# Adttil/crypto12381

Measured on AMD Instinct MI355X. Metric: G1 scalar-muls/s per MI355X (batch 2^20 per GPU), bit-exact vs CPU, higher is better.
Workload: dtype int64 accumulate over 14x28-bit signed limbs

## Files before the change

### crypto12381_amd/csrc/consts.hpp

```cpp
#pragma once
#include <cstdint>

namespace c12381 {

constexpr int NL = 14;
constexpr int LB = 28;
constexpr uint32_t LMASK = 0xfffffffu;
constexpr uint32_t FP_N0 = 0xffcfffdu;

C12381_CONST int32_t FP_P[14] = {0xfffaaab, 0xfefffff, 0x3ffffb9, 0xfffeb15, 0x6241eab, 0xa0f6b0f, 0xf6730d2, 0xf38512b, 0x4774b84, 0x4bacd76, 0xba7b643, 0xe69a4b1, 0x1ea397f, 0x001a011};
C12381_CONST int32_t FP_R1[14] = {0x347fcb8, 0xd800000, 0x002b119, 0x0cde6d2, 0xc7212e0, 0x83a2090, 0x037669f, 0xda0f73e, 0x9b09b42, 0x1297bb0, 0x515d98f, 0x012ca7c, 0x659fcfa, 0x000577a};
C12381_CONST int32_t FP_R2[14] = {0x10370ed, 0x6d1c345, 0xe243d62, 0xec45c53, 0x3b1d65a, 0x093317d, 0xb4f36a0, 0x5d74088, 0xc10ea72, 0x865d118, 0x7320a75, 0xfd5cd50, 0xcc8a759, 0x000c8d4};
C12381_CONST int32_t SG_P30[13] = {0x3fffaaab, 0x27fbffff, 0x153ffffb, 0x2affffac, 0x30f6241e, 0x034a83da, 0x112bf673, 0x12e13ce1, 0x2cd76477, 0x1ed90d2e, 0x29a4b1ba, 0x3a8e5ff9, 0x001a0111};
constexpr uint32_t SG_PINV30 = 0x30003u;
C12381_CONST int32_t FP_B3[14] = {0x760834a, 0x2200002, 0x8204dc2, 0x9a6fbad, 0x910a528, 0xe9ab0aa, 0x3ca6dd4, 0x51af490, 0xb58b018, 0x47c315a, 0x5b6c62e, 0x40e3470, 0x86368b8, 0x000d99a};
C12381_CONST int32_t FP_FOUR[14] = {0xd1ff2e0, 0x6000000, 0x00ac467, 0x3379b48, 0x1c84b80, 0x0e88243, 0x0dd9a7e, 0x683dcf8, 0x6c26d0b, 0x4a5eec2, 0x457663c, 0x04b29f1, 0x967f3e8, 0x0015de9};
C12381_CONST int32_t FP_HALF[14] = {0x1a3fe5c, 0xec00000, 0x001588c, 0x066f369, 0x6390970, 0xc1d1048, 0x01bb34f, 0x6d07b9f, 0x4d84da1, 0x894bdd8, 0x28aecc7, 0x009653e, 0x32cfe7d, 0x0002bbd};
C12381_CONST int32_t FP_INV3[14] = {0x66d1b5a, 0x4755555, 0x2ab902f, 0x0449454, 0x2e8c568, 0x972fce5, 0xa5742c1, 0x405dddc, 0x63510c4, 0x8dfb234, 0x977175c, 0x44cb14a, 0x8ba2553, 0x0013289};
C12381_CONST int32_t FP_BETA_A[14] = {0xa75929a, 0x681b798, 0x22a3e9d, 0xabc02bf, 0x4e5bb45, 0x55e6e7e, 0x4814117, 0x6d04f1b, 0xae3387d, 0x54acb0c, 0x0a4c74b, 0x56138b5, 0xb64e066, 0x00076f2};
C12381_CONST int32_t FP_BETA_B[14] = {0x2421b59, 0xbee4867, 0x1d31002, 0x4760184, 0x4cc5086, 0xc76dc00, 0xaae891b, 0xac70ad2, 0xfe377c4, 0xe4686b8, 0x5ed1568, 0x8f5a180, 0x02b5c1f, 0x000d1a4};
C12381_CONST int32_t FROB_F_A[14] = {0x9f1ba38, 0xed52b31, 0x3131f18, 0x932815a, 0x35bde3f, 0x7c4a4df, 0xc6f7465, 0x266b7cc, 0x2acd4ff, 0xcae398d, 0x243b688, 0xa613121, 0x72d376f, 0x0001c3e};
C12381_CONST int32_t FROB_F_B[14] = {0x60df073, 0x11ad4ce, 0x0ece0a1, 0x6cd69bb, 0x2c8406c, 0x24ac630, 0x2f7bc6d, 0xcd1995f, 0x1ca7685, 0x80c93e9, 0x963ffba, 0x4087390, 0xabd0210, 0x00183d2};
C12381_CONST int32_t FROB_F2_A[14] = {0x0000000, 0x0000000, 0x0000000, 0x0000000, 0x0000000, 0x0000000, 0x0000000, 0x0000000, 0x0000000, 0x0000000, 0x0000000, 0x0000000, 0x0000000, 0x0000000};
C12381_CONST int32_t FROB_F2_B[14] = {0x2421b59, 0xbee4867, 0x1d31002, 0x4760184, 0x4cc5086, 0xc76dc00, 0xaae891b, 0xac70ad2, 0xfe377c4, 0xe4686b8, 0x5ed1568, 0x8f5a180, 0x02b5c1f, 0x000d1a4};
C12381_CONST int32_t FROB_F3_A[14] = {0x33e2f27, 0x32a25aa, 0x27ca1d2, 0xc1e049e, 0xc3f707a, 0x055ca94, 0x2010b7b, 0x3b93794, 0xd5a86aa, 0xa544de3, 0x556a044, 0x9c66da5, 0x38ec515, 0x000cea3};
C12381_CONST int32_t FROB_F3_B[14] = {0x33e2f27, 0x32a25aa, 0x27ca1d2, 0xc1e049e, 0xc3f707a, 0x055ca94, 0x2010b7b, 0x3b93794, 0xd5a86aa, 0xa544de3, 0x556a044, 0x9c66da5, 0x38ec515, 0x000cea3};
C12381_CONST int32_t PSI1_X_A[14] = {0x0000000, 0x0000000, 0x0000000, 0x0000000, 0x0000000, 0x0000000, 0x0000000, 0x0000000, 0x0000000, 0x0000000, 0x0000000, 0x0000000, 0x0000000, 0x0000000};
C12381_CONST int32_t PSI1_X_B[14] = {0x58a1811, 0x96e4867, 0x1d5c11c, 0x543e856, 0x13e6366, 0x4b0fc91, 0xae5efbb, 0x8680210, 0x9941307, 0xf700269, 0xb02eef7, 0x9086bfc, 0x6855919, 0x001291e};
C12381_CONST int32_t PSI1_Y_A[14] = {0xcc17b84, 0xcc5da55, 0x1835de7, 0x3e1e677, 0x9e4ae31, 0x9b9a07a, 0xd662557, 0xb7f1997, 0x71cc4da, 0xa667f92, 0x65115fe, 0x4a3370c, 0xe5b746a, 0x000d16d};
C12381_CONST int32_t PSI1_Y_B[14] = {0x33e2f27, 0x32a25aa, 0x27ca1d2, 0xc1e049e, 0xc3f707a, 0x055ca94, 0x2010b7b, 0x3b93794, 0xd5a86aa, 0xa544de3, 0x556a044, 0x9c66da5, 0x38ec515, 0x000cea3};
C12381_CONST int32_t PSI3_X_A[14] = {0x0000000, 0x0000000, 0x0000000, 0x0000000, 0x0000000, 0x0000000, 0x0000000, 0x0000000, 0x0000000, 0x0000000, 0x0000000, 0x0000000, 0x0000000, 0x0000000};
C12381_CONST int32_t PSI3_X_B[14] = {0xcb7adf3, 0x26fffff, 0x3fd4ea0, 0xf320443, 0x9b20bcb, 0x1d54a7e, 0xf2fca33, 0x19759ed, 0xac6b042, 0x39151c5, 0x691dcb4, 0xe56da35, 0xb903c85, 0x0014896};
C12381_CONST int32_t PSI3_Y_A[14] = {0x33e2f27, 0x32a25aa, 0x27ca1d2, 0xc1e049e, 0xc3f707a, 0x055ca94, 0x2010b7b, 0x3b93794, 0xd5a86aa, 0xa544de3, 0x556a044, 0x9c66da5, 0x38ec515, 0x000cea3};
// ... 97 lines not shown
```

### crypto12381_amd/csrc/fp.hpp

```cpp
#pragma once
#include <cstdint>
#include <type_traits>
#include <utility>

#if defined(__HIPCC__)
#include <hip/hip_runtime.h>
#define C12381_HD __host__ __device__ __forceinline__
#define C12381_HDN __host__ __device__ __noinline__ inline
#define C12381_CONST __device__ constexpr
#else
#define C12381_HD inline
#define C12381_HDN inline
#define C12381_CONST constexpr
#endif

#if defined(__HIP_DEVICE_COMPILE__)
#define C12381_LIMB(x) c12381::limb_opaque(x)
namespace c12381 { __device__ __forceinline__ int32_t limb_opaque(int32_t v) { asm("" : "+v"(v)); return v; } }
#else
#define C12381_LIMB(x) (x)
#endif

#include "consts.hpp"

// ... 17 lines not shown

struct fp {
    int32_t l[NL];
#ifdef C12381_CHECK_BOUNDS
    double lb = 0, vb = 0;
#endif
};

#ifdef C12381_CHECK_BOUNDS
inline void bounds_fail(const char* what, double a, double b) {
    std::fprintf(stderr, "C12381 bound violation: %s (%.4g, %.4g)\n", what, a, b);
    void* frames[48];
    int nf = backtrace(frames, 48);
    backtrace_symbols_fd(frames, nf, 2);
    std::abort();
}
constexpr double P_OVER_R = 0.000396;
constexpr double TOP_PER_P = 106514.0;
inline void check_actual(const fp& a, const char* where) {
    for (int i = 0; i < NL; ++i)
        if (std::fabs((double)a.l[i]) > a.lb) bounds_fail(where, (double)a.l[i], a.lb);
}
inline void check_actual_vb(const fp& a, const char* where);
inline void set_inj_bounds(fp& r, double sum_lblb, double sum_vbvb, double inj_abs, double inj_lb, const char* where);
inline void set_bounds(fp& r, double lb, double vb, const char* where) {
    r.lb = lb; r.vb = vb;
    if (lb > 2147483648.0) bounds_fail("limb bound exceeds int32", lb, vb);
    check_actual(r, where);
}
#endif

C12381_HD void fp_add(fp& r, const fp& a, const fp& b) {
#pragma unroll
    for (int i = 0; i < NL; ++i) r.l[i] = a.l[i] + b.l[i];
    C12381_BOUNDS(set_bounds(r, a.lb + b.lb, a.vb + b.vb, "fp_add");)
}
C12381_HD void fp_sub(fp& r, const fp& a, const fp& b) {
#pragma unroll
    for (int i = 0; i < NL; ++i) r.l[i] = a.l[i] - b.l[i];
    C12381_BOUNDS(set_bounds(r, a.lb + b.lb, a.vb + b.vb, "fp_sub");)
}
C12381_HD void fp_neg(fp& r, const fp& a) {
#pragma unroll
    for (int i = 0; i < NL; ++i) r.l[i] = -a.l[i];
    C12381_BOUNDS(set_bounds(r, a.lb, a.vb, "fp_neg");)
}
C12381_HD void fp_dbl(fp& r, const fp& a) { fp_add(r, a, a); }
// ... 39 lines not shown
    t += (int64_t)a.l[NL - 1] * k;
    r.l[NL - 1] = (int32_t)t;
    C12381_BOUNDS({ double top = a.vb * k * TOP_PER_P + 2.0;
                    set_bounds(r, top > 268435456.0 ? top : 268435456.0, a.vb * k, "fp_mul_small"); })
}

C12381_HD void fp_weak_reduce(fp& r, const fp& a) {
    fp n;
    fp_norm1(n, a);
    const int32_t q = (int32_t)(((int64_t)n.l[NL - 1] * 40324 + ((int64_t)1 << 31)) >> 32);
    int64_t t = 0;
#pragma unroll
    for (int i = 0; i < NL - 1; ++i) {
        t += (int64_t)n.l[i] - (int64_t)q * FP_P[i];
        r.l[i] = C12381_LIMB((int32_t)((uint32_t)t & LMASK));
        t >>= LB;
    }
    t += (int64_t)n.l[NL - 1] - (int64_t)q * FP_P[NL - 1];
    r.l[NL - 1] = (int32_t)t;
    C12381_BOUNDS({ if (a.vb > 2400.0) bounds_fail("fp_weak_reduce input value bound", a.vb, 0);
                    set_bounds(r, 268435456.0, 1.6, "fp_weak_reduce"); })
}

#ifdef C12381_CHECK_BOUNDS
inline void check_mul_operands(const fp& a, const fp& b, const char* where) {
    check_actual(a, where); check_actual(b, where);
    double col = 14.0 * a.lb * b.lb + 14.0 * 72057594037927936.0 + 1099511627776.0;
    if (col >= 9223372036854775808.0) bounds_fail(where, a.lb, b.lb);
    if (a.vb * b.vb > 1.0e6) bounds_fail("fp_mul value bound", a.vb, b.vb);
}
#endif

C12381_HD void fp_mul(fp& r, const fp& a, const fp& b) {
    C12381_BOUNDS(check_mul_operands(a, b, "fp_mul");)
    C12381_COUNT(27, 1);
    int32_t m[NL];
    int32_t out[NL];
    int64_t acc = 0;
#pragma unroll
    for (int k = 0; k < NL; ++k) {
#pragma unroll
        for (int i = 0; i <= k; ++i) { acc += (int64_t)a.l[i] * b.l[k - i]; }
#pragma unroll
        for (int i = 0; i < k; ++i) { acc += (int64_t)m[i] * FP_P[k - i]; }
        m[k] = (int32_t)(((uint32_t)acc * FP_N0) & LMASK);
        acc += (int64_t)m[k] * FP_P[0];
        acc >>= LB;
    }
#pragma unroll
    for (int k = NL; k < 2 * NL - 1; ++k) {
#pragma unroll
        for (int i = k - NL + 1; i < NL; ++i) { acc += (int64_t)a.l[i] * b.l[k - i]; }
#pragma unroll
        for (int i = k - NL + 1; i < NL; ++i) { acc += (int64_t)m[i] * FP_P[k - i]; }
        out[k - NL] = C12381_LIMB((int32_t)((uint32_t)acc & LMASK));
        acc >>= LB;
    }
    out[NL - 1] = (int32_t)acc;
#pragma unroll
    for (int i = 0; i < NL; ++i) r.l[i] = out[i];
    C12381_BOUNDS({ double vb = a.vb * b.vb * P_OVER_R + 1.0;
                    double top = vb * TOP_PER_P + 2.0;
                    set_bounds(r, top > 268435456.0 ? top : 268435456.0, vb, "fp_mul"); })
}

C12381_HD void fp_sqr(fp& r, const fp& a) {
    C12381_BOUNDS(check_mul_operands(a, a, "fp_sqr");)
    C12381_COUNT(27, 1);
    int32_t m[NL];
    int32_t out[NL];
    int32_t a2[NL];
#pragma unroll
    for (int i = 0; i < NL; ++i) a2[i] = 2 * a.l[i];
    int64_t acc = 0;
#pragma unroll
    for (int k = 0; k < NL; ++k) {
#pragma unroll
        for (int i = 0; 2 * i < k; ++i) { acc += (int64_t)a2[i] * a.l[k - i]; }
        if ((k & 1) == 0) { acc += (int64_t)a.l[k / 2] * a.l[k / 2]; }
#pragma unroll
        for (int i = 0; i < k; ++i) { acc += (int64_t)m[i] * FP_P[k - i]; }
        m[k] = (int32_t)(((uint32_t)acc * FP_N0) & LMASK);
        acc += (int64_t)m[k] * FP_P[0];
        acc >>= LB;
    }
#pragma unroll
    for (int k = NL; k < 2 * NL - 1; ++k) {
#pragma unroll
        for (int i = k - NL + 1; 2 * i < k; ++i) { acc += (int64_t)a2[i] * a.l[k - i]; }
        if ((k & 1) == 0) { acc += (int64_t)a.l[k / 2] * a.l[k / 2]; }
#pragma unroll
        for (int i = k - NL + 1; i < NL; ++i) { acc += (int64_t)m[i] * FP_P[k - i]; }
        out[k - NL] = C12381_LIMB((int32_t)((uint32_t)acc & LMASK));
        acc >>= LB;
    }
    out[NL - 1] = (int32_t)acc;
#pragma unroll
    for (int i = 0; i < NL; ++i) r.l[i] = out[i];
    C12381_BOUNDS({ double vb = a.vb * a.vb * P_OVER_R + 1.0;
                    double top = vb * TOP_PER_P + 2.0;
                    set_bounds(r, top > 268435456.0 ? top : 268435456.0, vb, "fp_sqr"); })
}

C12381_HD void fp_col_acc(int64_t& acc, const fp& a, const fp& b, int k) {
    C12381_COUNT(1, 0);
#pragma unroll
    for (int i = 0; i < NL; ++i) {
        const int j = k - i;
        if (j >= 0 && j < NL) { acc += (int64_t)a.l[i] * b.l[j]; }
    }
}
C12381_HD void fp_col_sqr_acc(int64_t& acc, const fp& a, const fp& a2, const fp& ad, int k) {
    C12381_COUNT(1, 0);
#pragma unroll
    for (int i = 0; i < NL; ++i) {
        const int j = k - i;
        if (j > i && j < NL) { acc += (int64_t)a2.l[i] * a.l[j]; }
    }
    if ((k & 1) == 0 && k / 2 < NL) { acc += (int64_t)ad.l[k / 2] * a.l[k / 2]; }
}
C12381_HD void fp_raw_neg(fp& r, const fp& a) {
#pragma unroll
    for (int i = 0; i < NL; ++i) r.l[i] = -a.l[i];
    C12381_BOUNDS(r.lb = a.lb; r.vb = a.vb;)
}
C12381_HD void fp_raw_dbl(fp& r, const fp& a) {
#pragma unroll
    for (int i = 0; i < NL; ++i) r.l[i] = 2 * a.l[i];
    C12381_BOUNDS(r.lb = 2 * a.lb; r.vb = 2 * a.vb;)
}
C12381_HD void fp_raw_neg_dbl(fp& r, const fp& a) {
#pragma unroll
    for (int i = 0; i < NL; ++i) r.l[i] = -2 * a.l[i];
    C12381_BOUNDS(r.lb = 2 * a.lb; r.vb = 2 * a.vb;)
}
template <class ColFn>
C12381_HD void fp_reduce_cols(fp& r, ColFn col) {
    C12381_COUNT(0, 1);
    int32_t m[NL];
    int32_t out[NL];
    int64_t acc = 0;
#pragma unroll
    for (int k = 0; k < NL; ++k) {
        col(k, acc);
#pragma unroll
        for (int i = 0; i < k; ++i) { acc += (int64_t)m[i] * FP_P[k - i]; }
        m[k] = (int32_t)(((uint32_t)acc * FP_N0) & LMASK);
        acc += (int64_t)m[k] * FP_P[0];
        acc >>= LB;
    }
#pragma unroll
    for (int k = NL; k < 2 * NL - 1; ++k) {
        col(k, acc);
#pragma unroll
        for (int i = k - NL + 1; i < NL; ++i) { acc += (int64_t)m[i] * FP_P[k - i]; }
        out[k - NL] = C12381_LIMB((int32_t)((uint32_t)acc & LMASK));
        acc >>= LB;
    }
    out[NL - 1] = (int32_t)acc;
#pragma unroll
    for (int i = 0; i < NL; ++i) r.l[i] = out[i];
}
template <int... Ks, class Fn>
C12381_HD void fp_static_for(std::integer_sequence<int, Ks...>, Fn&& fn) { (fn(std::integral_constant<int, Ks>{}), ...); }
template <class ColFn>
C12381_HD void fp_reduce_cols_static(fp& r, ColFn col) {
    C12381_COUNT(0, 1);
    int32_t m[NL];
    int32_t out[NL];
    int64_t acc = 0;
    fp_static_for(std::make_integer_sequence<int, NL>{}, [&](auto kc) {
        constexpr int k = decltype(kc)::value;
        col(k, acc);
#pragma unroll
        for (int i = 0; i < k; ++i) { acc += (int64_t)m[i] * FP_P[k - i]; }
        m[k] = (int32_t)(((uint32_t)acc * FP_N0) & LMASK);
        acc += (int64_t)m[k] * FP_P[0];
        acc >>= LB;
    });
    fp_static_for(std::make_integer_sequence<int, NL - 1>{}, [&](auto kc) {
        constexpr int k = NL + decltype(kc)::value;
        col(k, acc);
#pragma unroll
        for (int i = k - NL + 1; i < NL; ++i) { acc += (int64_t)m[i] * FP_P[k - i]; }
        out[k - NL] = C12381_LIMB((int32_t)((uint32_t)acc & LMASK));
        acc >>= LB;
    });
    out[NL - 1] = (int32_t)acc;
#pragma unroll
    for (int i = 0; i < NL; ++i) r.l[i] = out[i];
}
C12381_HD void fp_inj(int64_t& acc, const fp& c, int i, int32_t k) { acc += (int64_t)c.l[i] * k; }
C12381_HD void fp_inj_p(int64_t& acc, int i, int32_t k) { acc += (int64_t)FP_P[i] * k; }
C12381_HD int32_t fp_quot_top(int32_t top) { return (int32_t)(((int64_t)top * 40324 + ((int64_t)1 << 31)) >> 32); }
#if defined(__HIP_DEVICE_COMPILE__)
C12381_HD int32_t fp_opaque_const(int32_t v) { asm("" : "+s"(v)); return v; }
#else
C12381_HD int32_t fp_opaque_const(int32_t v) { return v; }
#endif
template <class ColFn, class InjFn>
C12381_HD void fp_reduce_cols_inj(fp& r, ColFn col, InjFn inj) {
    C12381_COUNT(0, 1);
    int32_t m[NL];
    int32_t out[NL];
    int64_t acc = 0;
#pragma unroll
    for (int k = 0; k < NL; ++k) {
        col(k, acc);
#pragma unroll
        for (int i = 0; i < k; ++i) { acc += (int64_t)m[i] * FP_P[k - i]; }
        m[k] = (int32_t)(((uint32_t)acc * FP_N0) & LMASK);
        acc += (int64_t)m[k] * FP_P[0];
        acc >>= LB;
    }
#pragma unroll
    for (int k = NL; k < 2 * NL - 1; ++k) {
        col(k, acc);
        inj(k - NL, acc);
#pragma unroll
        for (int i = k - NL + 1; i < NL; ++i) { acc += (int64_t)m[i] * FP_P[k - i]; }
        out[k - NL] = C12381_LIMB((int32_t)((uint32_t)acc & LMASK));
        acc >>= LB;
    }
    inj(NL - 1, acc);
    out[NL - 1] = (int32_t)acc;
#pragma unroll
    for (int i = 0; i < NL; ++i) r.l[i] = out[i];
}
template <class InjFn>
C12381_HD void fp_mul_inj(fp& r, const fp& a, const fp& b, InjFn inj, double inj_vb, double inj_lb) {
    C12381_COUNT(27, 0);
    fp t;
    fp_reduce_cols_inj(t, [&](int k, int64_t& acc) {
#pragma unroll
        for (int i = 0; i < NL; ++i) { const int j = k - i; if (j >= 0 && j < NL) { acc += (int64_t)a.l[i] * b.l[j]; } }
    }, inj);
    (void)inj_vb; (void)inj_lb;
    C12381_BOUNDS({ check_actual(a, "fp_mul_inj"); check_actual(b, "fp_mul_inj"); set_inj_bounds(t, a.lb * b.lb, a.vb * b.vb, inj_vb, inj_lb, "fp_mul_inj"); })
    r = t;
}
template <class InjFn>
C12381_HD void fp_sqr_inj(fp& r, const fp& a, InjFn inj, double inj_vb, double inj_lb) {
    C12381_COUNT(27, 0);
    fp t, a2;
    fp_raw_dbl(a2, a);
    fp_reduce_cols_inj(t, [&](int k, int64_t& acc) {
#pragma unroll
        for (int i = 0; i < NL; ++i) { const int j = k - i; if (j > i && j < NL) { acc += (int64_t)a2.l[i] * a.l[j]; } }
        if ((k & 1) == 0 && k / 2 < NL) { acc += (int64_t)a.l[k / 2] * a.l[k / 2]; }
    }, inj);
    (void)inj_vb; (void)inj_lb;
    C12381_BOUNDS({ check_actual(a, "fp_sqr_inj"); set_inj_bounds(t, a.lb * a.lb, a.vb * a.vb, inj_vb, inj_lb, "fp_sqr_inj"); })
    r = t;
}
C12381_HD void fp_norm1_dbl(fp& r, const fp& a) {
    int32_t c[NL];
#pragma unroll
    for (int i = 0; i < NL - 1; ++i) c[i] = a.l[i] >> (LB - 1);
    const int32_t t13 = 2 * a.l[NL - 1] + c[NL - 2];
#pragma unroll
    for (int i = NL - 2; i >= 1; --i) r.l[i] = C12381_LIMB((int32_t)(((uint32_t)a.l[i] << 1) & LMASK)) + c[i - 1];
    r.l[0] = C12381_LIMB((int32_t)(((uint32_t)a.l[0] << 1) & LMASK));
    r.l[NL - 1] = t13;
    C12381_BOUNDS({ double top = 2 * a.vb * TOP_PER_P + 6.0 + std::floor(2 * a.lb / 268435456.0);
                    double lb = 268435456.0 + std::floor(2 * a.lb / 268435456.0) + 1.0;
                    set_bounds(r, lb > top ? lb : top, 2 * a.vb, "fp_norm1_dbl"); })
}

C12381_HD void fp_lincomb3p(fp& r, const fp& a, int32_t k0, const fp& b, int32_t k1, const fp& c, int32_t k2, int32_t kp, double vb) {
    int64_t t = 0;
    int32_t out[NL];
#pragma unroll
    for (int i = 0; i < NL - 1; ++i) {
        t += (int64_t)a.l[i] * k0; t += (int64_t)b.l[i] * k1; t += (int64_t)c.l[i] * k2; t += (int64_t)FP_P[i] * kp;
        out[i] = C12381_LIMB((int32_t)((uint32_t)t & LMASK));
        t >>= LB;
    }
    t += (int64_t)a.l[NL - 1] * k0; t += (int64_t)b.l[NL - 1] * k1; t += (int64_t)c.l[NL - 1] * k2; t += (int64_t)FP_P[NL - 1] * kp;
    out[NL - 1] = (int32_t)t;
#pragma unroll
    for (int i = 0; i < NL; ++i) r.l[i] = out[i];
    (void)vb;
    C12381_BOUNDS({ double top = vb * TOP_PER_P + 2.0;
                    set_bounds(r, top > 268435456.0 ? top : 268435456.0, vb, "fp_lincomb3p"); check_actual_vb(r, "fp_lincomb3p value"); })
}

template <bool SUB>
C12381_HD void fp_mul2(fp& r, const fp& a, const fp& b, const fp& c, const fp& d);

#ifdef C12381_CHECK_BOUNDS
inline void set_lazy_bounds(fp& r, double sum_lblb, double sum_vbvb, const char* where) {
    double col = 14.0 * sum_lblb + 14.0 * 72057594037927936.0 + 1099511627776.0;
    if (col >= 9223372036854775808.0) bounds_fail(where, sum_lblb, sum_vbvb);
    if (sum_vbvb > 1.0e6) bounds_fail("lazy form value bound", sum_vbvb, 0);
    double vb = sum_vbvb * P_OVER_R + 1.0;
    double top = vb * TOP_PER_P + 2.0;
    set_bounds(r, top > 268435456.0 ? top : 268435456.0, vb, where);
}
inline void set_inj_bounds(fp& r, double sum_lblb, double sum_vbvb, double inj_abs, double inj_lb, const char* where) {
    double col = 14.0 * sum_lblb + 14.0 * 72057594037927936.0 + 1099511627776.0 + inj_lb;
    if (col >= 9223372036854775808.0) bounds_fail(where, sum_lblb, inj_lb);
    if (sum_vbvb > 1.0e6) bounds_fail("injected form value bound", sum_vbvb, 0);
    double vb = sum_vbvb * P_OVER_R + 1.0 + inj_abs;
    double top = vb * TOP_PER_P + 2.0;
    set_bounds(r, top > 268435456.0 ? top : 268435456.0, vb, where);
    check_actual_vb(r, where);
}
inline double fp_actual_vb(const fp& a) {
    long double v = 0, w = 1;
    for (int i = 0; i < NL; ++i) { v += (long double)a.l[i] * w; w *= 268435456.0L; }
    long double pp = 0; w = 1;
    for (int i = 0; i < NL; ++i) { pp += (long double)FP_P[i] * w; w *= 268435456.0L; }
    return (double)fabsl(v / pp);
}
inline void check_actual_vb(const fp& a, const char* where) { const double v = fp_actual_vb(a); if (v > a.vb * 1.0000001 + 1e-9) bounds_fail(where, v, a.vb); }
#endif

template <bool SUB>
C12381_HD void fp_mul2(fp& r, const fp& a, const fp& b, const fp& c, const fp& d) {
    fp t, cs;
    if (SUB) fp_raw_neg(cs, c); else cs = c;
    fp_reduce_cols(t, [&](int k, int64_t& acc) { fp_col_acc(acc, a, b, k); fp_col_acc(acc, cs, d, k); });
    C12381_BOUNDS({ check_actual(a, "fp_mul2"); check_actual(b, "fp_mul2"); check_actual(c, "fp_mul2"); check_actual(d, "fp_mul2");
                    set_lazy_bounds(t, a.lb * b.lb + c.lb * d.lb, a.vb * b.vb + c.vb * d.vb, "fp_mul2"); })
    r = t;
}

C12381_HD void fp_from_mont_canonical(fp& r, const fp& a) {
    fp one;
    fp_zero(one);
    one.l[0] = 1;
    C12381_BOUNDS(one.lb = 1; one.vb = 1e-100;)
    fp t;
    fp_mul(t, a, one);
    bool eqp = true;
#pragma unroll
    for (int i = 0; i < NL; ++i) eqp = eqp && (t.l[i] == FP_P[i]);
#pragma unroll
    for (int i = 0; i < NL; ++i) r.l[i] = eqp ? 0 : t.l[i];
    C12381_BOUNDS(r.lb = 268435456.0; r.vb = 1.0;)
}
C12381_HD bool fp_is_zero(const fp& a) {
    fp t;
    fp_from_mont_canonical(t, a);
    int32_t o = 0;
#pragma unroll
    for (int i = 0; i < NL; ++i) o |= t.l[i];
    return o == 0;
}
C12381_HD bool fp_equal(const fp& a, const fp& b) {
    fp d;
    fp_sub(d, a, b);
    return fp_is_zero(d);
}

C12381_HD void fp_from_words_be(fp& r, const uint32_t (&w)[12]) {
    fp t;
// ... 193 lines not shown
```

### crypto12381_amd/csrc/g1.hpp

```cpp
#pragma once
#include "fp.hpp"

namespace c12381 {

struct g1p { fp x, y, z; };

C12381_HD void g1_set_inf(g1p& p) { fp_zero(p.x); fp_one(p.y); fp_zero(p.z); }
C12381_HD bool g1_is_inf(const g1p& p) { return fp_is_zero(p.z); }
C12381_HD void g1_norm1(g1p& r, const g1p& p) { fp_norm1(r.x, p.x); fp_norm1(r.y, p.y); fp_norm1(r.z, p.z); }

C12381_HD void g1_dbl(g1p& p) {
    fp t0, t1, t2, z8, u, y3, x3, z3;
    const int32_t cm3 = fp_opaque_const(-3);
    fp_mul(t1, p.y, p.z);
    fp_sqr(t2, p.z);
    fp_mul_small(t2, t2, 12);
    fp_sqr_inj(u, p.y, [&](int i, int64_t& acc) { fp_inj(acc, t2, i, cm3); }, C12381_BV(3 * t2.vb), C12381_BV(3 * t2.lb));
    fp_dbl(t0, t2); fp_add(t0, t0, t2); fp_add(t0, t0, u);
    fp_mul_small(z8, t0, 8);
    fp_add(y3, t0, t2);
    fp_mul(z3, t1, z8);
    fp_mul2<false>(y3, u, y3, t2, z8);
    fp_mul(t1, p.x, p.y);
    fp_mul(x3, u, t1);
// ... 14 lines not shown
        fp_add(sa, p.y, p.z); fp_add(sb, q.y, q.z);
        fp_mul_inj(t4, sa, sb, [&](int i, int64_t& acc) { fp_inj(acc, t1, i, cm1); fp_inj(acc, t2, i, cm1); }, C12381_BV(t1.vb + t2.vb), C12381_BV(t1.lb + t2.lb));
    }
    fp_add(x3, p.x, p.z); fp_add(y3, q.x, q.z); fp_mul(x3, x3, y3);
    fp_add(y3, t0, t2); fp_sub(y3, x3, y3);
    fp_mul_small(t0, t0, 3);
    fp_mul_small(t2, t2, 12);
    fp_add(z3, t1, t2); fp_sub(t1, t1, t2);
    fp_mul_small(y3, y3, 12);
    fp_mul2<true>(p.x, t3, t1, y3, t4);
    fp_mul2<false>(p.y, y3, t0, t1, z3);
    fp_mul2<false>(p.z, z3, t4, t0, t3);
}

C12381_HD void g1_endo_x2(g1p& r, const g1p& p) {
    fp beta;
    fp_set_const(beta, FP_BETA_A);
    fp_mul(r.x, p.x, beta);
    fp_neg(r.y, p.y);
    r.z = p.z;
}

struct g1j { fp x, y, z; };

C12381_HD void g1j_dbl(g1j& p) {
    fp a, b, c, d, e, xb, x3, y3, z3, y2;
    const int32_t cm1 = fp_opaque_const(-1), cm4 = fp_opaque_const(-4), cm8 = fp_opaque_const(-8);
    fp_raw_dbl(y2, p.y);
    fp_mul(z3, y2, p.z);
    fp_sqr(a, p.x);
    fp_sqr(b, p.y);
    fp_sqr(c, b);
    fp_add(xb, p.x, b);
    fp_sqr_inj(d, xb, [&](int i, int64_t& acc) { fp_inj(acc, a, i, cm1); fp_inj(acc, c, i, cm1); },
               C12381_BV(a.vb + c.vb), C12381_BV(a.lb + c.lb));
    fp_mul_small(e, a, 3);
    fp_sqr_inj(x3, e, [&](int i, int64_t& acc) { fp_inj(acc, d, i, cm4); }, C12381_BV(4 * d.vb), C12381_BV(4 * d.lb));
    fp_raw_dbl(d, d);
    fp_sub(d, d, x3);
    fp_mul_inj(y3, e, d, [&](int i, int64_t& acc) { fp_inj(acc, c, i, cm8); }, C12381_BV(8 * c.vb), C12381_BV(8 * c.lb));
    p.x = x3; p.y = y3; p.z = z3;
}

C12381_HD void g1j_madd(g1j& r, const g1j& p, const fp& x2, const fp& y2) {
    fp zz, zzz, u2, s2, h, s, hh, hhh, v, x3, y3, z3, vx;
    const int32_t cm1 = fp_opaque_const(-1), cm2 = fp_opaque_const(-2);
    fp_sqr(zz, p.z);
    fp_mul(u2, x2, zz);
    fp_mul(zzz, p.z, zz);
    fp_mul(s2, y2, zzz);
    fp_sub(h, u2, p.x);
    fp_sub(s, s2, p.y);
    fp_mul(z3, p.z, h);
    fp_sqr(hh, h);
    fp_mul(hhh, h, hh);
    fp_mul(v, p.x, hh);
    fp_sqr_inj(x3, s, [&](int i, int64_t& acc) { fp_inj(acc, hhh, i, cm1); fp_inj(acc, v, i, cm2); },
               C12381_BV(hhh.vb + 2 * v.vb), C12381_BV(hhh.lb + 2 * v.lb));
    fp_sub(vx, v, x3);
    fp_mul2<true>(y3, s, vx, p.y, hhh);
    r.x = x3; r.y = y3; r.z = z3;
}

C12381_HD void g1j_dblu(fp& x2, fp& y2, fp& x1, fp& y1, const fp& x, const fp& y) {
    fp a, b, c, d, e, xb, dd;
    const int32_t cm1 = fp_opaque_const(-1), cm4 = fp_opaque_const(-4), cm8 = fp_opaque_const(-8);
    fp_sqr(a, x);
    fp_sqr(b, y);
    fp_sqr(c, b);
    fp_add(xb, x, b);
    fp_sqr_inj(d, xb, [&](int i, int64_t& acc) { fp_inj(acc, a, i, cm1); fp_inj(acc, c, i, cm1); },
               C12381_BV(a.vb + c.vb), C12381_BV(a.lb + c.lb));
    fp_mul_small(e, a, 3);
    fp_sqr_inj(x2, e, [&](int i, int64_t& acc) { fp_inj(acc, d, i, cm4); }, C12381_BV(4 * d.vb), C12381_BV(4 * d.lb));
    fp_raw_dbl(dd, d);
    fp_sub(dd, dd, x2);
    fp_mul_inj(y2, e, dd, [&](int i, int64_t& acc) { fp_inj(acc, c, i, cm8); }, C12381_BV(8 * c.vb), C12381_BV(8 * c.lb));
    fp_mul_small(x1, d, 2);
    fp_mul_small(y1, c, 8);
}
C12381_HD void g1j_zaddu(fp& x3, fp& y3, fp& x1, fp& y1, fp& h, const fp& x2, const fp& y2) {
    fp c, w1, w2, sd, dw, a1, wx;
    const int32_t cm1 = fp_opaque_const(-1);
// ... 337 lines not shown
    rec_field(a, w, 0, vb_cap); rec_field(b, w, NL, vb_cap); rec_field(c, w, 2 * NL, vb_cap);
}
C12381_HD void tab_load_xy(fp& x, fp& y, const int32_t* ent) {
    int32_t w[G1_ENT_DWORDS];
    tab_load_q4<0, 7>(w, ent);
    rec_field(x, w, 0, 4.0); rec_field(y, w, NL, 4.0);
}
C12381_HD void tab_load_ybx(fp& y, fp& bx, const int32_t* ent) {
    int32_t w[G1_ENT_DWORDS];
    tab_load_q4<3, 8>(w, ent);
    rec_field(y, w, NL, 4.0); rec_field(bx, w, 2 * NL, 4.0);
}
struct alignas(8) d2 { int32_t v[2]; };
C12381_HD void tab_store_zt(int32_t* lane_tab, const fp& zt) {
#pragma unroll
    for (int j = 0; j < NL / 2; ++j) { d2 t; t.v[0] = zt.l[2 * j]; t.v[1] = zt.l[2 * j + 1]; *reinterpret_cast<d2*>(lane_tab + j * G1_ENT_DWORDS + 42) = t; }
}
C12381_HD void tab_load_zt(fp& zt, const int32_t* lane_tab) {
#pragma unroll
    for (int j = 0; j < NL / 2; ++j) { const d2 t = *reinterpret_cast<const d2*>(lane_tab + j * G1_ENT_DWORDS + 42); zt.l[2 * j] = t.v[0]; zt.l[2 * j + 1] = t.v[1]; }
    C12381_BOUNDS(zt.lb = G1_REC_LB; zt.vb = 4.0; check_actual(zt, "tab_load_zt");)
}

C12381_HD void g1j_add_digit(g1j& acc, bool& acc_inf, const fp& x, const fp& y, int d, bool endo) {
    fp ny, ys, one;
    fp_neg(ny, y);
    fp_select(ys, (d < 0) != endo, ny, y);
    g1j r;
    g1j_madd(r, acc, x, ys);
    fp_one(one);
    fp_select(r.x, acc_inf, x, r.x); fp_select(r.y, acc_inf, ys, r.y); fp_select(r.z, acc_inf, one, r.z);
    const bool keep = d == 0;
    fp_select(acc.x, keep, acc.x, r.x); fp_select(acc.y, keep, acc.y, r.y); fp_select(acc.z, keep, acc.z, r.z);
    acc_inf = acc_inf && keep;
}

C12381_HD bool g1_scalar_mul(g1p& acc, const fp& px, const fp& py, bool p_is_inf, const uint32_t (&kin)[8], int32_t* lane_tab) {
    uint32_t k[8];
#pragma unroll
    for (int i = 0; i < 8; ++i) k[i] = kin[i];
    scalar_mod_r(k);
    uint32_t k0[4], k1[4], kb0[5], kb1[5];
    scalar_glv_split(k0, k1, k);
    glv_bias(kb0, k0);
    glv_bias(kb1, k1);

    fp beta;
    fp_set_const(beta, FP_BETA_A);
    {
        fp x1, y1, xj, yj, xn, yn, h, hn, bx;
        g1j_dblu(xj, yj, x1, y1, px, py);
#pragma unroll 1
        for (int j = 2; j < G1_TAB; ++j) {
            g1j_zaddu(xn, yn, x1, y1, h, xj, yj);
// ... 45 lines not shown
        const int d0 = glv_digit(kb0, w), d1 = glv_digit(kb1, w);
        fp x0, y0, x1, y1;
        tab_load_xy(x0, y0, g1_digit_entry(lane_tab, d0));
#if defined(__HIP_DEVICE_COMPILE__)
        __builtin_amdgcn_sched_barrier(0);
#endif
        g1j_dbl(a); g1j_dbl(a); g1j_dbl(a); g1j_dbl(a);
        if (G1_WIN == 5) g1j_dbl(a);
        tab_load_ybx(y1, x1, g1_digit_entry(lane_tab, d1));
#if defined(__HIP_DEVICE_COMPILE__)
        __builtin_amdgcn_sched_barrier(0);
#endif
        g1j_add_digit(a, acc_inf, x0, y0, d0, false);
        g1j_add_digit(a, acc_inf, x1, y1, d1, true);
    }

    fp zt, z, z2;
    tab_load_zt(zt, lane_tab);
    fp_mul(z, a.z, zt);
    const bool inf = acc_inf || p_is_inf;
    const bool exc = !inf && fp_is_zero(z);
    fp_sqr(z2, z);
    fp_mul(acc.x, a.x, z);
    acc.y = a.y;
    fp_mul(acc.z, z2, z);
    {
        g1p o;
        g1_set_inf(o);
        fp_select(acc.x, inf, o.x, acc.x); fp_select(acc.y, inf, o.y, acc.y); fp_select(acc.z, inf, o.z, acc.z);
    }
    if (exc) g1_scalar_mul_complete(acc, px, py, p_is_inf, kin, lane_tab);
    return exc;
}
C12381_HD bool scalar_below_x2(const uint32_t (&kin)[8]) {
    uint32_t k[8];
#pragma unroll
    for (int i = 0; i < 8; ++i) k[i] = kin[i];
    scalar_mod_r(k);
    uint64_t bw = 0;
#pragma unroll
    for (int i = 0; i < 4; ++i) { uint64_t t = (uint64_t)k[i] - GLV_X2[i] - bw; bw = (t >> 32) & 1; }
    return (k[4] | k[5] | k[6] | k[7]) == 0u && bw == 1;
}

C12381_HD void g1_to_affine(fp& ax, fp& ay, const g1p& p, const fp& zinv) {
    fp_mul(ax, p.x, zinv);
    fp_mul(ay, p.y, zinv);
}
// ... 14 lines not shown
```

Before: 44.76 million.

## Use unmasked 32-bit Montgomery quotient digits with balanced modulus limbs in G1 loop

Adds a Montgomery reduction variant that computes the quotient digit as a plain 32-bit product with a 32-bit inverse, skipping the mask, and uses balanced signed limbs of p. The point doubling and mixed addition in the main loop use this variant. The output value bound loosens, so the final y coordinate is now weak-reduced. Separately, the infinity-accumulator select in add_digit is skipped when no lane in the wave has acc_inf set, which adds a wave vote.

```diff
diff --git a/crypto12381_amd/csrc/consts.hpp b/crypto12381_amd/csrc/consts.hpp
--- a/crypto12381_amd/csrc/consts.hpp
+++ b/crypto12381_amd/csrc/consts.hpp
@@ -9,6 +9,8 @@
 constexpr uint32_t FP_N0 = 0xffcfffdu;
 
 C12381_CONST int32_t FP_P[14] = {0xfffaaab, 0xfefffff, 0x3ffffb9, 0xfffeb15, 0x6241eab, 0xa0f6b0f, 0xf6730d2, 0xf38512b, 0x4774b84, 0x4bacd76, 0xba7b643, 0xe69a4b1, 0x1ea397f, 0x001a011};
+C12381_CONST int32_t FP_PB[14] = {-0x0005555, -0x0100000, 0x3ffffba, -0x00014eb, 0x6241eac, -0x5f094f1, -0x098cf2d, -0x0c7aed4, 0x4774b85, 0x4bacd76, -0x45849bd, -0x1965b4e, 0x1ea3980, 0x001a011};
+constexpr uint32_t FP_N0_32 = 0xfffcfffdu;
 C12381_CONST int32_t FP_R1[14] = {0x347fcb8, 0xd800000, 0x002b119, 0x0cde6d2, 0xc7212e0, 0x83a2090, 0x037669f, 0xda0f73e, 0x9b09b42, 0x1297bb0, 0x515d98f, 0x012ca7c, 0x659fcfa, 0x000577a};
 C12381_CONST int32_t FP_R2[14] = {0x10370ed, 0x6d1c345, 0xe243d62, 0xec45c53, 0x3b1d65a, 0x093317d, 0xb4f36a0, 0x5d74088, 0xc10ea72, 0x865d118, 0x7320a75, 0xfd5cd50, 0xcc8a759, 0x000c8d4};
 C12381_CONST int32_t SG_P30[13] = {0x3fffaaab, 0x27fbffff, 0x153ffffb, 0x2affffac, 0x30f6241e, 0x034a83da, 0x112bf673, 0x12e13ce1, 0x2cd76477, 0x1ed90d2e, 0x29a4b1ba, 0x3a8e5ff9, 0x001a0111};
diff --git a/crypto12381_amd/csrc/fp.hpp b/crypto12381_amd/csrc/fp.hpp
--- a/crypto12381_amd/csrc/fp.hpp
+++ b/crypto12381_amd/csrc/fp.hpp
@@ -63,7 +63,7 @@
         if (std::fabs((double)a.l[i]) > a.lb) bounds_fail(where, (double)a.l[i], a.lb);
 }
 inline void check_actual_vb(const fp& a, const char* where);
-inline void set_inj_bounds(fp& r, double sum_lblb, double sum_vbvb, double inj_abs, double inj_lb, const char* where);
+inline void set_inj_bounds(fp& r, double sum_lblb, double sum_vbvb, double inj_abs, double inj_lb, const char* where, bool um = false);
 inline void set_bounds(fp& r, double lb, double vb, const char* where) {
     r.lb = lb; r.vb = vb;
     if (lb > 2147483648.0) bounds_fail("limb bound exceeds int32", lb, vb);
@@ -149,19 +149,42 @@
                     set_bounds(r, 268435456.0, 1.6, "fp_weak_reduce"); })
 }
 
+constexpr bool FP_UM = true;
 #ifdef C12381_CHECK_BOUNDS
-inline void check_mul_operands(const fp& a, const fp& b, const char* where) {
+constexpr double redc_col(bool um) { return um ? 14.0 * 288230376151711744.0 : 14.0 * 72057594037927936.0; }
+constexpr double redc_vb(bool um) { return um ? 8.000001 : 1.0; }
+inline void check_mul_operands(const fp& a, const fp& b, const char* where, bool um = false) {
     check_actual(a, where); check_actual(b, where);
-    double col = 14.0 * a.lb * b.lb + 14.0 * 72057594037927936.0 + 1099511627776.0;
+    double col = 14.0 * a.lb * b.lb + redc_col(um) + 1099511627776.0;
     if (col >= 9223372036854775808.0) bounds_fail(where, a.lb, b.lb);
     if (a.vb * b.vb > 1.0e6) bounds_fail("fp_mul value bound", a.vb, b.vb);
 }
 #endif
-
+template <bool UM>
+C12381_HD int32_t fp_qdigit(int64_t acc) {
+    if (UM) return (int32_t)((uint32_t)acc * FP_N0_32);
+    return (int32_t)(((uint32_t)acc * FP_N0) & LMASK);
+}
+#if defined(__HIP_DEVICE_COMPILE__)
+C12381_HD int32_t fp_pdigit_opaque(int32_t v) { asm("" : "+s"(v)); return v; }
+#else
+C12381_HD int32_t fp_pdigit_opaque(int32_t v) { return v; }
+#endif
+template <bool UM>
+struct fp_pdigits {
+    int32_t d[NL];
+    C12381_HD fp_pdigits() {
+#pragma unroll
+        for (int i = 0; i < NL; ++i) d[i] = UM ? FP_PB[i] : FP_P[i];
+        if (UM) d[1] = fp_pdigit_opaque(FP_PB[1]);
+    }
+};
+template <bool UM = false>
 C12381_HD void fp_mul(fp& r, const fp& a, const fp& b) {
-    C12381_BOUNDS(check_mul_operands(a, b, "fp_mul");)
+    C12381_BOUNDS(check_mul_operands(a, b, "fp_mul", UM);)
     C12381_COUNT(27, 1);
     int32_t m[NL];
+    const fp_pdigits<UM> pd;
     int32_t out[NL];
     int64_t acc = 0;
 #pragma unroll
@@ -169,9 +192,9 @@
 #pragma unroll
         for (int i = 0; i <= k; ++i) { acc += (int64_t)a.l[i] * b.l[k - i]; }
 #pragma unroll
-        for (int i = 0; i < k; ++i) { acc += (int64_t)m[i] * FP_P[k - i]; }
-        m[k] = (int32_t)(((uint32_t)acc * FP_N0) & LMASK);
-        acc += (int64_t)m[k] * FP_P[0];
+        for (int i = 0; i < k; ++i) { acc += (int64_t)m[i] * pd.d[k - i]; }
+        m[k] = fp_qdigit<UM>(acc);
+        acc += (int64_t)m[k] * pd.d[0];
         acc >>= LB;
     }
 #pragma unroll
@@ -179,22 +202,24 @@
 #pragma unroll
         for (int i = k - NL + 1; i < NL; ++i) { acc += (int64_t)a.l[i] * b.l[k - i]; }
 #pragma unroll
-        for (int i = k - NL + 1; i < NL; ++i) { acc += (int64_t)m[i] * FP_P[k - i]; }
+        for (int i = k - NL + 1; i < NL; ++i) { acc += (int64_t)m[i] * pd.d[k - i]; }
         out[k - NL] = C12381_LIMB((int32_t)((uint32_t)acc & LMASK));
         acc >>= LB;
     }
     out[NL - 1] = (int32_t)acc;
 #pragma unroll
     for (int i = 0; i < NL; ++i) r.l[i] = out[i];
-    C12381_BOUNDS({ double vb = a.vb * b.vb * P_OVER_R + 1.0;
+    C12381_BOUNDS({ double vb = a.vb * b.vb * P_OVER_R + redc_vb(UM);
                     double top = vb * TOP_PER_P + 2.0;
                     set_bounds(r, top > 268435456.0 ? top : 268435456.0, vb, "fp_mul"); })
 }
 
+template <bool UM = false>
 C12381_HD void fp_sqr(fp& r, const fp& a) {
-    C12381_BOUNDS(check_mul_operands(a, a, "fp_sqr");)
+    C12381_BOUNDS(check_mul_operands(a, a, "fp_sqr", UM);)
     C12381_COUNT(27, 1);
     int32_t m[NL];
+    const fp_pdigits<UM> pd;
     int32_t out[NL];
     int32_t a2[NL];
 #pragma unroll
@@ -206,9 +231,9 @@
         for (int i = 0; 2 * i < k; ++i) { acc += (int64_t)a2[i] * a.l[k - i]; }
         if ((k & 1) == 0) { acc += (int64_t)a.l[k / 2] * a.l[k / 2]; }
 #pragma unroll
-        for (int i = 0; i < k; ++i) { acc += (int64_t)m[i] * FP_P[k - i]; }
-        m[k] = (int32_t)(((uint32_t)acc * FP_N0) & LMASK);
-        acc += (int64_t)m[k] * FP_P[0];
+        for (int i = 0; i < k; ++i) { acc += (int64_t)m[i] * pd.d[k - i]; }
+        m[k] = fp_qdigit<UM>(acc);
+        acc += (int64_t)m[k] * pd.d[0];
         acc >>= LB;
     }
 #pragma unroll
@@ -217,14 +242,14 @@
         for (int i = k - NL + 1; 2 * i < k; ++i) { acc += (int64_t)a2[i] * a.l[k - i]; }
         if ((k & 1) == 0) { acc += (int64_t)a.l[k / 2] * a.l[k / 2]; }
 #pragma unroll
-        for (int i = k - NL + 1; i < NL; ++i) { acc += (int64_t)m[i] * FP_P[k - i]; }
+        for (int i = k - NL + 1; i < NL; ++i) { acc += (int64_t)m[i] * pd.d[k - i]; }
         out[k - NL] = C12381_LIMB((int32_t)((uint32_t)acc & LMASK));
         acc >>= LB;
     }
     out[NL - 1] = (int32_t)acc;
 #pragma unroll
     for (int i = 0; i < NL; ++i) r.l[i] = out[i];
-    C12381_BOUNDS({ double vb = a.vb * a.vb * P_OVER_R + 1.0;
+    C12381_BOUNDS({ double vb = a.vb * a.vb * P_OVER_R + redc_vb(UM);
                     double top = vb * TOP_PER_P + 2.0;
                     set_bounds(r, top > 268435456.0 ? top : 268435456.0, vb, "fp_sqr"); })
 }
@@ -261,26 +286,27 @@
     for (int i = 0; i < NL; ++i) r.l[i] = -2 * a.l[i];
     C12381_BOUNDS(r.lb = 2 * a.lb; r.vb = 2 * a.vb;)
 }
-template <class ColFn>
+template <bool UM = false, class ColFn>
 C12381_HD void fp_reduce_cols(fp& r, ColFn col) {
     C12381_COUNT(0, 1);
     int32_t m[NL];
+    const fp_pdigits<UM> pd;
     int32_t out[NL];
     int64_t acc = 0;
 #pragma unroll
     for (int k = 0; k < NL; ++k) {
         col(k, acc);
 #pragma unroll
-        for (int i = 0; i < k; ++i) { acc += (int64_t)m[i] * FP_P[k - i]; }
-        m[k] = (int32_t)(((uint32_t)acc * FP_N0) & LMASK);
-        acc += (int64_t)m[k] * FP_P[0];
+        for (int i = 0; i < k; ++i) { acc += (int64_t)m[i] * pd.d[k - i]; }
+        m[k] = fp_qdigit<UM>(acc);
+        acc += (int64_t)m[k] * pd.d[0];
         acc >>= LB;
     }
 #pragma unroll
     for (int k = NL; k < 2 * NL - 1; ++k) {
         col(k, acc);
 #pragma unroll
-        for (int i = k - NL + 1; i < NL; ++i) { acc += (int64_t)m[i] * FP_P[k - i]; }
+        for (int i = k - NL + 1; i < NL; ++i) { acc += (int64_t)m[i] * pd.d[k - i]; }
         out[k - NL] = C12381_LIMB((int32_t)((uint32_t)acc & LMASK));
         acc >>= LB;
     }
@@ -290,26 +316,27 @@
 }
 template <int... Ks, class Fn>
 C12381_HD void fp_static_for(std::integer_sequence<int, Ks...>, Fn&& fn) { (fn(std::integral_constant<int, Ks>{}), ...); }
-template <class ColFn>
+template <bool UM = false, class ColFn>
 C12381_HD void fp_reduce_cols_static(fp& r, ColFn col) {
     C12381_COUNT(0, 1);
     int32_t m[NL];
+    const fp_pdigits<UM> pd;
     int32_t out[NL];
     int64_t acc = 0;
     fp_static_for(std::make_integer_sequence<int, NL>{}, [&](auto kc) {
         constexpr int k = decltype(kc)::value;
         col(k, acc);
 #pragma unroll
-        for (int i = 0; i < k; ++i) { acc += (int64_t)m[i] * FP_P[k - i]; }
-        m[k] = (int32_t)(((uint32_t)acc * FP_N0) & LMASK);
-        acc += (int64_t)m[k] * FP_P[0];
+        for (int i = 0; i < k; ++i) { acc += (int64_t)m[i] * pd.d[k - i]; }
+        m[k] = fp_qdigit<UM>(acc);
+        acc += (int64_t)m[k] * pd.d[0];
         acc >>= LB;
     });
     fp_static_for(std::make_integer_sequence<int, NL - 1>{}, [&](auto kc) {
         constexpr int k = NL + decltype(kc)::value;
         col(k, acc);
 #pragma unroll
-        for (int i = k - NL + 1; i < NL; ++i) { acc += (int64_t)m[i] * FP_P[k - i]; }
+        for (int i = k - NL + 1; i < NL; ++i) { acc += (int64_t)m[i] * pd.d[k - i]; }
         out[k - NL] = C12381_LIMB((int32_t)((uint32_t)acc & LMASK));
         acc >>= LB;
     });
@@ -325,19 +352,20 @@
 #else
 C12381_HD int32_t fp_opaque_const(int32_t v) { return v; }
 #endif
-template <class ColFn, class InjFn>
+template <bool UM = false, class ColFn, class InjFn>
 C12381_HD void fp_reduce_cols_inj(fp& r, ColFn col, InjFn inj) {
     C12381_COUNT(0, 1);
     int32_t m[NL];
+    const fp_pdigits<UM> pd;
     int32_t out[NL];
     int64_t acc = 0;
 #pragma unroll
     for (int k = 0; k < NL; ++k) {
         col(k, acc);
 #pragma unroll
-        for (int i = 0; i < k; ++i) { acc += (int64_t)m[i] * FP_P[k - i]; }
-        m[k] = (int32_t)(((uint32_t)acc * FP_N0) & LMASK);
-        acc += (int64_t)m[k] * FP_P[0];
+        for (int i = 0; i < k; ++i) { acc += (int64_t)m[i] * pd.d[k - i]; }
+        m[k] = fp_qdigit<UM>(acc);
+        acc += (int64_t)m[k] * pd.d[0];
         acc >>= LB;
     }
 #pragma unroll
@@ -345,7 +373,7 @@
         col(k, acc);
         inj(k - NL, acc);
 #pragma unroll
-        for (int i = k - NL + 1; i < NL; ++i) { acc += (int64_t)m[i] * FP_P[k - i]; }
+        for (int i = k - NL + 1; i < NL; ++i) { acc += (int64_t)m[i] * pd.d[k - i]; }
         out[k - NL] = C12381_LIMB((int32_t)((uint32_t)acc & LMASK));
         acc >>= LB;
     }
@@ -354,30 +382,30 @@
 #pragma unroll
     for (int i = 0; i < NL; ++i) r.l[i] = out[i];
 }
-template <class InjFn>
+template <bool UM = false, class InjFn>
 C12381_HD void fp_mul_inj(fp& r, const fp& a, const fp& b, InjFn inj, double inj_vb, double inj_lb) {
     C12381_COUNT(27, 0);
     fp t;
-    fp_reduce_cols_inj(t, [&](int k, int64_t& acc) {
+    fp_reduce_cols_inj<UM>(t, [&](int k, int64_t& acc) {
 #pragma unroll
         for (int i = 0; i < NL; ++i) { const int j = k - i; if (j >= 0 && j < NL) { acc += (int64_t)a.l[i] * b.l[j]; } }
     }, inj);
     (void)inj_vb; (void)inj_lb;
-    C12381_BOUNDS({ check_actual(a, "fp_mul_inj"); check_actual(b, "fp_mul_inj"); set_inj_bounds(t, a.lb * b.lb, a.vb * b.vb, inj_vb, inj_lb, "fp_mul_inj"); })
+    C12381_BOUNDS({ check_actual(a, "fp_mul_inj"); check_actual(b, "fp_mul_inj"); set_inj_bounds(t, a.lb * b.lb, a.vb * b.vb, inj_vb, inj_lb, "fp_mul_inj", UM); })
     r = t;
 }
-template <class InjFn>
+template <bool UM = false, class InjFn>
 C12381_HD void fp_sqr_inj(fp& r, const fp& a, InjFn inj, double inj_vb, double inj_lb) {
     C12381_COUNT(27, 0);
     fp t, a2;
     fp_raw_dbl(a2, a);
-    fp_reduce_cols_inj(t, [&](int k, int64_t& acc) {
+    fp_reduce_cols_inj<UM>(t, [&](int k, int64_t& acc) {
 #pragma unroll
         for (int i = 0; i < NL; ++i) { const int j = k - i; if (j > i && j < NL) { acc += (int64_t)a2.l[i] * a.l[j]; } }
         if ((k & 1) == 0 && k / 2 < NL) { acc += (int64_t)a.l[k / 2] * a.l[k / 2]; }
     }, inj);
     (void)inj_vb; (void)inj_lb;
-    C12381_BOUNDS({ check_actual(a, "fp_sqr_inj"); set_inj_bounds(t, a.lb * a.lb, a.vb * a.vb, inj_vb, inj_lb, "fp_sqr_inj"); })
+    C12381_BOUNDS({ check_actual(a, "fp_sqr_inj"); set_inj_bounds(t, a.lb * a.lb, a.vb * a.vb, inj_vb, inj_lb, "fp_sqr_inj", UM); })
     r = t;
 }
 C12381_HD void fp_norm1_dbl(fp& r, const fp& a) {
@@ -412,23 +440,23 @@
                     set_bounds(r, top > 268435456.0 ? top : 268435456.0, vb, "fp_lincomb3p"); check_actual_vb(r, "fp_lincomb3p value"); })
 }
 
-template <bool SUB>
+template <bool SUB, bool UM = false>
 C12381_HD void fp_mul2(fp& r, const fp& a, const fp& b, const fp& c, const fp& d);
 
 #ifdef C12381_CHECK_BOUNDS
-inline void set_lazy_bounds(fp& r, double sum_lblb, double sum_vbvb, const char* where) {
-    double col = 14.0 * sum_lblb + 14.0 * 72057594037927936.0 + 1099511627776.0;
+inline void set_lazy_bounds(fp& r, double sum_lblb, double sum_vbvb, const char* where, bool um = false) {
+    double col = 14.0 * sum_lblb + redc_col(um) + 1099511627776.0;
     if (col >= 9223372036854775808.0) bounds_fail(where, sum_lblb, sum_vbvb);
     if (sum_vbvb > 1.0e6) bounds_fail("lazy form value bound", sum_vbvb, 0);
-    double vb = sum_vbvb * P_OVER_R + 1.0;
+    double vb = sum_vbvb * P_OVER_R + redc_vb(um);
     double top = vb * TOP_PER_P + 2.0;
     set_bounds(r, top > 268435456.0 ? top : 268435456.0, vb, where);
 }
-inline void set_inj_bounds(fp& r, double sum_lblb, double sum_vbvb, double inj_abs, double inj_lb, const char* where) {
-    double col = 14.0 * sum_lblb + 14.0 * 72057594037927936.0 + 1099511627776.0 + inj_lb;
+inline void set_inj_bounds(fp& r, double sum_lblb, double sum_vbvb, double inj_abs, double inj_lb, const char* where, bool um) {
+    double col = 14.0 * sum_lblb + redc_col(um) + 1099511627776.0 + inj_lb;
     if (col >= 9223372036854775808.0) bounds_fail(where, sum_lblb, inj_lb);
     if (sum_vbvb > 1.0e6) bounds_fail("injected form value bound", sum_vbvb, 0);
-    double vb = sum_vbvb * P_OVER_R + 1.0 + inj_abs;
+    double vb = sum_vbvb * P_OVER_R + redc_vb(um) + inj_abs;
     double top = vb * TOP_PER_P + 2.0;
     set_bounds(r, top > 268435456.0 ? top : 268435456.0, vb, where);
     check_actual_vb(r, where);
@@ -443,13 +471,13 @@
 inline void check_actual_vb(const fp& a, const char* where) { const double v = fp_actual_vb(a); if (v > a.vb * 1.0000001 + 1e-9) bounds_fail(where, v, a.vb); }
 #endif
 
-template <bool SUB>
+template <bool SUB, bool UM>
 C12381_HD void fp_mul2(fp& r, const fp& a, const fp& b, const fp& c, const fp& d) {
     fp t, cs;
     if (SUB) fp_raw_neg(cs, c); else cs = c;
-    fp_reduce_cols(t, [&](int k, int64_t& acc) { fp_col_acc(acc, a, b, k); fp_col_acc(acc, cs, d, k); });
+    fp_reduce_cols<UM>(t, [&](int k, int64_t& acc) { fp_col_acc(acc, a, b, k); fp_col_acc(acc, cs, d, k); });
     C12381_BOUNDS({ check_actual(a, "fp_mul2"); check_actual(b, "fp_mul2"); check_actual(c, "fp_mul2"); check_actual(d, "fp_mul2");
-                    set_lazy_bounds(t, a.lb * b.lb + c.lb * d.lb, a.vb * b.vb + c.vb * d.vb, "fp_mul2"); })
+                    set_lazy_bounds(t, a.lb * b.lb + c.lb * d.lb, a.vb * b.vb + c.vb * d.vb, "fp_mul2", UM); })
     r = t;
 }
 
@@ -459,7 +487,7 @@
     one.l[0] = 1;
     C12381_BOUNDS(one.lb = 1; one.vb = 1e-100;)
     fp t;
-    fp_mul(t, a, one);
+    fp_mul<false>(t, a, one);
     bool eqp = true;
 #pragma unroll
     for (int i = 0; i < NL; ++i) eqp = eqp && (t.l[i] == FP_P[i]);
diff --git a/crypto12381_amd/csrc/g1.hpp b/crypto12381_amd/csrc/g1.hpp
--- a/crypto12381_amd/csrc/g1.hpp
+++ b/crypto12381_amd/csrc/g1.hpp
@@ -60,43 +60,44 @@
 }
 
 struct g1j { fp x, y, z; };
+constexpr bool G1_LOOP_UM = true;
 
 C12381_HD void g1j_dbl(g1j& p) {
     fp a, b, c, d, e, xb, x3, y3, z3, y2;
     const int32_t cm1 = fp_opaque_const(-1), cm4 = fp_opaque_const(-4), cm8 = fp_opaque_const(-8);
     fp_raw_dbl(y2, p.y);
-    fp_mul(z3, y2, p.z);
+    fp_mul<G1_LOOP_UM>(z3, y2, p.z);
     fp_sqr(a, p.x);
     fp_sqr(b, p.y);
-    fp_sqr(c, b);
+    fp_sqr<G1_LOOP_UM>(c, b);
     fp_add(xb, p.x, b);
-    fp_sqr_inj(d, xb, [&](int i, int64_t& acc) { fp_inj(acc, a, i, cm1); fp_inj(acc, c, i, cm1); },
+    fp_sqr_inj<G1_LOOP_UM>(d, xb, [&](int i, int64_t& acc) { fp_inj(acc, a, i, cm1); fp_inj(acc, c, i, cm1); },
                C12381_BV(a.vb + c.vb), C12381_BV(a.lb + c.lb));
     fp_mul_small(e, a, 3);
-    fp_sqr_inj(x3, e, [&](int i, int64_t& acc) { fp_inj(acc, d, i, cm4); }, C12381_BV(4 * d.vb), C12381_BV(4 * d.lb));
+    fp_sqr_inj<G1_LOOP_UM>(x3, e, [&](int i, int64_t& acc) { fp_inj(acc, d, i, cm4); }, C12381_BV(4 * d.vb), C12381_BV(4 * d.lb));
     fp_raw_dbl(d, d);
     fp_sub(d, d, x3);
-    fp_mul_inj(y3, e, d, [&](int i, int64_t& acc) { fp_inj(acc, c, i, cm8); }, C12381_BV(8 * c.vb), C12381_BV(8 * c.lb));
+    fp_mul_inj<G1_LOOP_UM>(y3, e, d, [&](int i, int64_t& acc) { fp_inj(acc, c, i, cm8); }, C12381_BV(8 * c.vb), C12381_BV(8 * c.lb));
     p.x = x3; p.y = y3; p.z = z3;
 }
 
 C12381_HD void g1j_madd(g1j& r, const g1j& p, const fp& x2, const fp& y2) {
     fp zz, zzz, u2, s2, h, s, hh, hhh, v, x3, y3, z3, vx;
     const int32_t cm1 = fp_opaque_const(-1), cm2 = fp_opaque_const(-2);
-    fp_sqr(zz, p.z);
-    fp_mul(u2, x2, zz);
-    fp_mul(zzz, p.z, zz);
-    fp_mul(s2, y2, zzz);
+    fp_sqr<G1_LOOP_UM>(zz, p.z);
+    fp_mul<G1_LOOP_UM>(u2, x2, zz);
+    fp_mul<G1_LOOP_UM>(zzz, p.z, zz);
+    fp_mul<G1_LOOP_UM>(s2, y2, zzz);
     fp_sub(h, u2, p.x);
     fp_sub(s, s2, p.y);
-    fp_mul(z3, p.z, h);
-    fp_sqr(hh, h);
-    fp_mul(hhh, h, hh);
-    fp_mul(v, p.x, hh);
-    fp_sqr_inj(x3, s, [&](int i, int64_t& acc) { fp_inj(acc, hhh, i, cm1); fp_inj(acc, v, i, cm2); },
+    fp_mul<G1_LOOP_UM>(z3, p.z, h);
+    fp_sqr<G1_LOOP_UM>(hh, h);
+    fp_mul<G1_LOOP_UM>(hhh, h, hh);
+    fp_mul<G1_LOOP_UM>(v, p.x, hh);
+    fp_sqr_inj<G1_LOOP_UM>(x3, s, [&](int i, int64_t& acc) { fp_inj(acc, hhh, i, cm1); fp_inj(acc, v, i, cm2); },
                C12381_BV(hhh.vb + 2 * v.vb), C12381_BV(hhh.lb + 2 * v.lb));
     fp_sub(vx, v, x3);
-    fp_mul2<true>(y3, s, vx, p.y, hhh);
+    fp_mul2<true, G1_LOOP_UM>(y3, s, vx, p.y, hhh);
     r.x = x3; r.y = y3; r.z = z3;
 }
 
@@ -480,14 +481,23 @@
     C12381_BOUNDS(zt.lb = G1_REC_LB; zt.vb = 4.0; check_actual(zt, "tab_load_zt");)
 }
 
+C12381_HD bool wave_any(bool c) {
+#if defined(__HIP_DEVICE_COMPILE__)
+    return __any(c);
+#else
+    return c;
+#endif
+}
 C12381_HD void g1j_add_digit(g1j& acc, bool& acc_inf, const fp& x, const fp& y, int d, bool endo) {
     fp ny, ys, one;
     fp_neg(ny, y);
     fp_select(ys, (d < 0) != endo, ny, y);
     g1j r;
     g1j_madd(r, acc, x, ys);
-    fp_one(one);
-    fp_select(r.x, acc_inf, x, r.x); fp_select(r.y, acc_inf, ys, r.y); fp_select(r.z, acc_inf, one, r.z);
+    if (wave_any(acc_inf)) {
+        fp_one(one);
+        fp_select(r.x, acc_inf, x, r.x); fp_select(r.y, acc_inf, ys, r.y); fp_select(r.z, acc_inf, one, r.z);
+    }
     const bool keep = d == 0;
     fp_select(acc.x, keep, acc.x, r.x); fp_select(acc.y, keep, acc.y, r.y); fp_select(acc.z, keep, acc.z, r.z);
     acc_inf = acc_inf && keep;
@@ -579,8 +589,9 @@
     const bool exc = !inf && fp_is_zero(z);
     fp_sqr(z2, z);
     fp_mul(acc.x, a.x, z);
-    acc.y = a.y;
+    fp_weak_reduce(acc.y, a.y);
     fp_mul(acc.z, z2, z);
+    C12381_BOUNDS(for (const fp* e : {&acc.x, &acc.y, &acc.z}) if (e->vb > 4.0) bounds_fail("g1_scalar_mul output value bound", e->vb, 4.0);)
     {
         g1p o;
         g1_set_inf(o);
```

Result: no change. 45.00 million (median of 6 runs) (+0.6%).
